# marian42/shapegan

Hardware: AMD Instinct MI355X
Metric: GAN train steps/sec @32^3 voxels (train_wgan.py 5 critic + 1 generator updates, batch 64/GPU) (higher is better)
Workload: dtype f32; 1 GPU; train_wgan.py 32^3 voxel WGAN, fp32, batch=64 synthetic SDF grids (BASELINE configs[1]); global_batch=64, per_gpu_batch=64, parallelism=dp1

## Files before the change

### include/shapegan_hip.h

```cpp
#ifndef SHAPEGAN_HIP_H
#define SHAPEGAN_HIP_H

#include <stddef.h>
#include <stdint.h>

#ifdef __cplusplus
extern "C" {
#endif

#define SG_ABI_VERSION 8

typedef struct ihipStream_t* hipStream_t;

#define SG_ACT_NONE_C 0
#define SG_ACT_LEAKY_C 1
#define SG_ACT_RELU_C 2
#define SG_ACT_TANH_C 3
#define SG_ACT_SIGMOID_C 4

int sg_abi_version(void);
const char* sg_last_error(void);

size_t sg_conv3d_k4s2p1_fwd_workspace_bytes(int batch, int Cin, int Cout, int OD, int OH, int OW);
int sg_conv3d_k4s2p1_fwd(const float* x, const float* w, const float* bias, float* y, int batch, int Cin, int Cin_total,
                         int Cx, int Cout, int ID, int IH, int IW, int act, float slope, void* workspace,
                         size_t workspace_bytes, hipStream_t stream);
int sg_conv3d_k4s2p1_fwd_keep(const float* x, const float* w, const float* bias, float* y, int batch, int Cin, int Cin_total,
                              int Cx, int Cout, int ID, int IH, int IW, int act, float slope, void* workspace,
                              size_t workspace_bytes, int weights_unchanged, hipStream_t stream);
long long sg_conv3d_k4s2p1_image_layout(int kind, const int* dims, size_t workspace_bytes);
int sg_conv3d_k4s2p1_pack_images(int n, const int* kinds, const float* const* weights, void* const* workspaces,
                                 const size_t* workspace_bytes, const int* dims, int* served, hipStream_t stream);
int sg_conv3d_k4s2p1_fwd_impl(const float* x, const float* w, const float* bias, float* y, int batch, int Cin,
                              int Cin_total, int Cx, int Cout, int ID, int IH, int IW, int act, float slope,
                              void* workspace, size_t workspace_bytes, int impl, int debug, hipStream_t stream);
size_t sg_conv3d_k4s2p1_dgrad_workspace_bytes(int Cout, int Cin);
size_t sg_conv3d_k4s2p1_dgrad_workspace_bytes_for(int batch, int Cin, int Cout, int OD, int OH, int OW);
int sg_conv3d_k4s2p1_dgrad(const float* dy, const float* w, const float* bias, float* dx, int batch, int Cin,
                           int Cin_total, int Cx, int Cout, int ID, int IH, int IW, int act, float slope,
                           void* workspace, size_t workspace_bytes, hipStream_t stream);
int sg_conv3d_k4s2p1_dgrad_keep(const float* dy, const float* w, const float* bias, float* dx, int batch, int Cin,
                                int Cin_total, int Cx, int Cout, int ID, int IH, int IW, int act, float slope,
                                void* workspace, size_t workspace_bytes, int weights_unchanged, hipStream_t stream);
int sg_conv3d_k4s2p1_dgrad_impl(const float* dy, const float* w, const float* bias, float* dx, int batch, int Cin,
                                int Cin_total, int Cx, int Cout, int ID, int IH, int IW, int act, float slope,
                                void* workspace, size_t workspace_bytes, int impl, hipStream_t stream);
size_t sg_conv3d_k4s2p1_wgrad_workspace_bytes(int batch, int Cin, int Cout, int OD, int OH, int OW);
int sg_conv3d_k4s2p1_wgrad_impl(const float* dy, const float* x, float* dw, int batch, int Cin, int Cin_total, int Cx,
                                int Cout, int ID, int IH, int IW, void* workspace, size_t workspace_bytes, int impl,
                                hipStream_t stream);
int sg_conv3d_k4s2p1_wgrad(const float* dy, const float* x, float* dw, int batch, int Cin, int Cin_total, int Cx,
                           int Cout, int ID, int IH, int IW, void* workspace, size_t workspace_bytes,
                           hipStream_t stream);
int sg_conv3d_k4s2p1_wgrad_dy_image(int batch, int Cin, int Cout, int OD, int OH, int OW, size_t workspace_bytes, int* mt_total,
                                    long* nslice);
int sg_act_bwd_rowsum_pack8(const float* y, const float* dy, float* dz, float* rowsum, void* dz_image, long N, int C, long nslice,
                            int act, float slope, hipStream_t stream);
int sg_conv3d_k4s2p1_wgrad_prepacked(const float* dy, const float* x, float* dw, int batch, int Cin, int Cin_total, int Cx,
                                     int Cout, int ID, int IH, int IW, void* workspace, size_t workspace_bytes, hipStream_t stream);
int sg_conv3d_k4s2p1_wgrad_act_eligible(int batch, int Cin, int Cout, int OD, int OH, int OW, int act);
int sg_conv3d_k4s2p1_wgrad_act(const float* dy, const float* y, const float* x, float* dw, float* db, int batch, int Cin,
                               int Cin_total, int Cx, int Cout, int ID, int IH, int IW, int act, float slope, void* workspace,
                               size_t workspace_bytes, hipStream_t stream);

int sg_convT3d_k4s2p1_fwd(const float* x, const float* w, const float* bias, float* y, int batch, int Cin_T, int Cout_T,
                          int ID, int IH, int IW, int act, float slope, void* workspace, size_t workspace_bytes,
                          hipStream_t stream);
int sg_convT3d_k4s2p1_to1_pre_eligible(int batch, int C, int ID, int IH, int IW);
int sg_convT3d_k4s2p1_to1_pre(const float* x, const float* w, const float* bias, float* y, const float* in_scale,
                              const float* in_shift, int in_act, float in_slope, int batch, int C, int ID, int IH, int IW, int act,
                              float slope, hipStream_t stream);
int sg_convT3d_k4s2p1_to1_pre_impl(const float* x, const float* w, const float* bias, float* y, const float* in_scale,
                                   const float* in_shift, int in_act, float in_slope, int batch, int C, int ID, int IH, int IW,
                                   int act, float slope, int form, hipStream_t stream);
int sg_convT3d_k4s2p1_to1_pre_grouped(const float* x, const float* w, const float* bias, float* y, const float* in_scale,
                                      const float* in_shift, int in_act, float in_slope, int batch, int C, int ID, int IH, int IW,
                                      int act, float slope, int samples_per_group, long y_group_stride, hipStream_t stream);
int sg_convT3d_k4s2p1_dgrad(const float* dy, const float* w, float* dx, int batch, int Cin_T, int Cout_T, int ID, int IH,
                            int IW, void* workspace, size_t workspace_bytes, hipStream_t stream);
int sg_convT3d_k4s2p1_wgrad(const float* dy, const float* x, float* dw, int batch, int Cin_T, int Cout_T, int ID, int IH,
                            int IW, void* workspace, size_t workspace_bytes, hipStream_t stream);

size_t sg_gemm_workspace_bytes(int M, int N);
int sg_gemm(const float* A, long sai, long sak, const float* B, long sbk, long sbj, float* C, long sci, long scj,
            const float* bias_i, const float* bias_j, int bias_j_shift, int M, int N, int K, int act, float slope,
            void* workspace, size_t workspace_bytes, hipStream_t stream);
#define SG_GEMM_KIND_SKELETON 0
#define SG_GEMM_KIND_GEMM128 1
#define SG_GEMM_KIND_GEMM128_SPLIT 2
#define SG_GEMM_KIND_PERSISTENT 3
#define SG_GEMM_FINALIZE_NONE 0
#define SG_GEMM_FINALIZE_FLAT 1
#define SG_GEMM_FINALIZE_DEEP 2
int sg_gemm_plan(const void* A, long sai, long sak, const void* B, long sbk, long sbj, long sci, long scj, int has_bias_i, int M, int N,
                 int K, const void* workspace, size_t workspace_bytes, long* plan);
int sg_gemm_nt_plan(int batch, int M, int N, long K, long* plan);
size_t sg_gemm_nt_workspace_bytes(int M, int N, long K);
int sg_gemm_nt(const float* A, long lda, const float* B, long ldb, float* C, long ldc, int M, int N, long K, void* workspace,
               size_t workspace_bytes, hipStream_t stream);
// ... 413 lines not shown
```

### shapegan_amd/csrc/conv3d.hip

```cpp
#include "mfma_tile.h"
#include <stdlib.h>

#include "conv_common.h"
#include "../../include/shapegan_hip.h"

namespace sg {

struct PatchCtx {
    int base;
    int mask;
    __device__ __forceinline__ void set(const ConvGeom& g, uint32_t pos) {
        int n, od, oh, ow;
        decode_pos(g, pos, n, od, oh, ow);
        const int id0 = 2 * od - 1, ih0 = 2 * oh - 1, iw0 = 2 * ow - 1;
        base = n * g.Cx * g.ID * g.IH * g.IW + (id0 * g.IH + ih0) * g.IW + iw0;
        int m = 0;
#pragma unroll
        for (int t = 0; t < 4; ++t) {
            if ((unsigned)(id0 + t) < (unsigned)g.ID) m |= 1 << t;
            if ((unsigned)(ih0 + t) < (unsigned)g.IH) m |= 1 << (4 + t);
            if ((unsigned)(iw0 + t) < (unsigned)g.IW) m |= 1 << (8 + t);
        }
        mask = m;
    }
// ... 659 lines not shown

static bool kept_image_of_call(int kind, int batch, int Cin, int Cout, const ConvGeom& g, size_t workspace_bytes, ImageJob* image) {
    if (kind == 0) {
        const HaloFwdPlan p = halo_fwd_plan(batch, Cin, Cout, g, workspace_bytes);
        *image = p.image;
        return p.served;
    }
    const HaloDgradPlan p = halo_dgrad_plan(batch, Cin, Cout, g, workspace_bytes);
    *image = p.image;
    return p.served;
}

int sg_conv3d_k4s2p1_pack_images(int n, const int* kinds, const float* const* weights, void* const* workspaces,
                                 const size_t* workspace_bytes, const int* dims, int* served, hipStream_t stream) {
    SG_CHECK_ARG(n > 0 && n <= 8 && kinds && weights && workspaces && workspace_bytes && dims && served);
    PackJobs jobs;
    for (int i = 0; i < n; ++i) {
        const int* d = dims + 8 * i;
        const int batch = d[0], Cin = d[1], Cin_total = d[2], Cx = d[3], Cout = d[4];
        served[i] = 0;
        SG_CHECK_ARG(weights[i] && batch > 0 && Cin > 0 && Cin <= Cin_total && Cin <= Cx && Cout > 0 && (kinds[i] == 0 || kinds[i] == 1));
        ConvGeom g;
        if (make_geom(g, d[5], d[6], d[7], Cx, Cout)) SG_FAIL(SG_ERR_ARG, "sg_conv3d_k4s2p1_pack_images: bad spatial dims");
        if (check_sizes(g, batch, "sg_conv3d_k4s2p1_pack_images")) return SG_ERR_ARG;
        ImageJob image;
        if (!kept_image_of_call(kinds[i], batch, Cin, Cout, g, workspaces[i] ? workspace_bytes[i] : 0, &image)) continue;
        served[i] = jobs.add(image, weights[i], workspaces[i], Cout, Cin_total, Cin);
    }
    halo_pack_jobs_launch(jobs, stream);
    SG_CHECK_LAUNCH();
    return SG_OK;
}

long long sg_conv3d_k4s2p1_image_layout(int kind, const int* dims, size_t workspace_bytes) {
    if (!dims || (kind != 0 && kind != 1)) return 0;
    const int batch = dims[0], Cin = dims[1], Cin_total = dims[2], Cx = dims[3], Cout = dims[4];
    if (batch <= 0 || Cin <= 1 || Cin > Cin_total || Cin > Cx || Cout <= 0) return 0;
    ConvGeom g;
    if (make_geom(g, dims[5], dims[6], dims[7], Cx, Cout)) return 0;
    if ((long)batch * g.O3() >= (1L << 31) || (long)batch * g.I3() >= (1L << 31)) return 0;
    ImageJob j;
    if (!kept_image_of_call(kind, batch, Cin, Cout, g, workspace_bytes, &j)) return 0;
    unsigned long long h = 1469598103934665603ull;
    const long long f[7] = {j.kind + 1, Cout, Cin_total, Cin, j.nt, (long long)j.offset, 0x5347};
    for (long long v : f)
        for (int b = 0; b < 8; ++b) {
            h ^= (unsigned long long)(v >> (8 * b)) & 0xffull;
            h *= 1099511628211ull;
        }
    h &= 0x7fffffffffffffffull;
    return h ? (long long)h : 1;
}

int sg_conv3d_k4s2p1_dgrad_impl(const float* dy, const float* w, const float* bias, float* dx, int batch, int Cin,
                                int Cin_total, int Cx, int Cout, int ID, int IH, int IW, int act, float slope,
                                void* workspace, size_t workspace_bytes, int impl, hipStream_t stream) {
    HaloDgradForm form;
    SG_CHECK_ARG(dy && w && dx && batch > 0 && Cin > 0 && Cin <= Cin_total && Cin <= Cx && Cout > 0 &&
                 halo_dgrad_form_decode(impl, &form) && form.forced &&
                 (form.ppw == 0 || (!form.one_parity && (form.ppw == 2 || form.ppw == 4 || form.ppw == 8))));
    ConvGeom g;
    if (make_geom(g, ID, IH, IW, Cx, Cout)) SG_FAIL(SG_ERR_ARG, "sg_conv3d_k4s2p1_dgrad_impl: bad spatial dims");
    if (check_sizes(g, batch, "sg_conv3d_k4s2p1_dgrad_impl")) return SG_ERR_ARG;
    const HaloDgradPlan hp = halo_dgrad_plan(batch, Cin, Cout, g, workspace ? workspace_bytes : 0, form);
    if (!hp.served) SG_FAIL(SG_ERR_ARG, "sg_conv3d_k4s2p1_dgrad_impl: shape not eligible for the LDS-halo kernel");
    halo_dgrad_pack(hp, w, Cin, Cin_total, Cout, workspace, stream);
    halo_dgrad_launch(hp, dy, bias, dx, batch, Cin, Cout, g, act, slope, workspace, stream);
    SG_CHECK_LAUNCH();
    return SG_OK;
}

int sg_conv3d_k4s2p1_wgrad_impl(const float* dy, const float* x, float* dw, int batch, int Cin, int Cin_total, int Cx,
                                int Cout, int ID, int IH, int IW, void* workspace, size_t workspace_bytes, int impl,
                                hipStream_t stream) {
    SG_CHECK_ARG(dy && x && dw && batch > 0 && Cin > 0 && Cin <= Cin_total && Cin <= Cx && Cout > 0 && impl == 1);
    ConvGeom g;
    if (make_geom(g, ID, IH, IW, Cx, Cout)) SG_FAIL(SG_ERR_ARG, "sg_conv3d_k4s2p1_wgrad_impl: bad spatial dims");
    if (check_sizes(g, batch, "sg_conv3d_k4s2p1_wgrad_impl")) return SG_ERR_ARG;
    const HaloWgradPlan hp = halo_wgrad_plan(batch, Cin, Cout, g, workspace ? workspace_bytes : 0, true);
    if (!hp.served) SG_FAIL(SG_ERR_ARG, "sg_conv3d_k4s2p1_wgrad_impl: shape not eligible for the LDS-halo kernel");
    halo_wgrad_pack(hp, dy, Cout, g, workspace, stream);
    halo_wgrad_launch(hp, x, dw, Cin, Cin_total, Cout, g, workspace, stream);
    SG_CHECK_LAUNCH();
    return SG_OK;
}

int sg_conv3d_k4s2p1_wgrad_dy_image(int batch, int Cin, int Cout, int OD, int OH, int OW, size_t workspace_bytes, int* mt_total,
                                    long* nslice) {
    if (batch <= 0 || Cin <= 0 || Cout <= 0 || !mt_total || !nslice) return 0;
    ConvGeom g;
    if (make_geom(g, 2 * OD, 2 * OH, 2 * OW, Cin, Cout)) return 0;
    const HaloWgradPlan hp = halo_wgrad_plan(batch, Cin, Cout, g, workspace_bytes, false);
    if (!hp.producer_image) return 0;
    *mt_total = hp.dy_image.nt;
    *nslice = hp.nslice;
    return 1;
}
int sg_act_bwd_rowsum_pack8(const float* y, const float* dy, float* dz, float* rowsum, void* dz_image, long N, int C, long nslice,
                            int act, float slope, hipStream_t stream) {
    SG_CHECK_ARG(y && dy && dz && rowsum && dz_image && N > 0 && C > 0 && C % 128 == 0 && nslice == N * 8);
    SG_CHECK_ARG(act == SG_ACT_LEAKY || act == SG_ACT_RELU);
    SG_CHECK_ARG((((uintptr_t)y | (uintptr_t)dy | (uintptr_t)dz | (uintptr_t)dz_image) & 15) == 0);
    halo_act_bwd_pack8_launch(y, dy, dz, rowsum, dz_image, N * C, C, nslice, act, slope, stream);
    SG_CHECK_LAUNCH();
    return SG_OK;
}
// ... 130 lines not shown
```

### shapegan_amd/csrc/conv3d_halo.hip

```cpp
#include "conv_common.h"

#ifndef SG_RING
#define SG_RING 8
#endif
#ifndef SG_ABLATE
#define SG_ABLATE 0
#endif

namespace sg {

constexpr int kHD = 4, kHH = 18, kHWF = 18;
constexpr int kHWH = 10;
constexpr int kROWH = 2 * kHWH;
constexpr int kROWD = kHH * kROWH;
constexpr int kHS = kHD * kROWD;
constexpr int kCC = 4;

struct HaloFwdArgs {
    const float* x;
    const float4* wp;
    const float* bias;
    float* y;
    ConvGeom g;
    int Cin, Cout;
// ... 1111 lines not shown
#pragma unroll
            for (int i = 0; i < 4; ++i) b[i] = bq[i];
            if (c + 1 < kDCC) {
#pragma unroll
                for (int i = 0; i < 4; ++i) bq[i] = bb[CUR * kDBUF + (c + 1) * kDB + (H0 + i) * BX::PL];
            }
            if (c < kDCC / 2) {
#pragma unroll
                for (int f = 2 * c; f < 2 * c + 2; ++f) fv[f] = buf_load(dres, goff[f], dys + pshift);
            } else {
#pragma unroll
                for (int f = 2 * (c - kDCC / 2); f < 2 * (c - kDCC / 2) + 2; ++f) sdst[NXT * kDBUF + 256 * f] = fv[f];
            }
            __builtin_amdgcn_sched_barrier(0);
            const float av[2][2] = {{a_cur.x, a_cur.y}, {a_cur.z, a_cur.w}};
#pragma unroll
            for (int td = 0; td < 2; ++td)
#pragma unroll
                for (int qd = 0; qd < 4; ++qd) {
                    constexpr int kDead0 = 0, kDead1 = 4;
                    const int hd = qd + 1 - td;
                    if (hd == (PD ? kDead1 : kDead0)) continue;
#pragma unroll
                    for (int rh = 0; rh < 2; ++rh)
                        acc[rh][qd] = __builtin_amdgcn_mfma_f32_16x16x4f32(av[td][rh], b[hd - H0], acc[rh][qd], 0, 0, 0);
                }
            __builtin_amdgcn_sched_barrier(0);
        }
        wcur = wnext;
        __syncthreads();
    };
    auto run_parity = [&](auto pdtag, int par) __attribute__((always_inline)) {
        const bool more = par + 1 < par_end;
        const unsigned wlast = more ? (unsigned)(par + 1) * par_bytes : (unsigned)par * par_bytes + (unsigned)(nstage - 1) * kDCC * 1024u;
        const unsigned dlast = more ? 0u : (unsigned)(nstage - 1) * kDCC * chan_bytes;
        int s = 0;
        for (; s + 1 < nstage; s += 2) {
            stage(IntTag<0>(), pdtag, (unsigned)(s + 1) * kDCC * chan_bytes, wcur + kDCC * 1024u);
            const bool last = s + 2 == nstage;
            if (last && more) set_goff(par + 1);
            stage(IntTag<1>(), pdtag, last ? dlast : (unsigned)(s + 2) * kDCC * chan_bytes, last ? wlast : wcur + kDCC * 1024u);
        }
        if (s < nstage) stage(IntTag<0>(), pdtag, dlast, wlast);
    };
    for (int par = par0; par < par_end; ++par) {
        if ((par >> 2) & 1)
            run_parity(IntTag<1>(), par);
        else
            run_parity(IntTag<0>(), par);
        write_parity(par);
    }
}

size_t halo_dgrad_workspace_bytes(int Cin, int Cout) { return (size_t)8 * ((Cin + 63) / 64) * 64 * Cout * 8 * sizeof(float); }

bool halo_dgrad_form_decode(int impl, HaloDgradForm* form) {
    form->forced = (impl & 1) != 0;
    form->one_parity = (impl & 2) != 0;
    form->ppw = (impl >> 2) & 15;
    form->rows64_dskip = (impl & 64) != 0;
    return (impl & ~127) == 0;
}

HaloDgradPlan halo_dgrad_plan(int batch, int Cin, int Cout, const ConvGeom& g, size_t workspace_bytes, HaloDgradForm form) {
    HaloDgradPlan p = HaloDgradPlan();
    const bool mode1 = g.OD == 4 && g.OH == 4 && g.OW == 4;
    if (!mode1 && (g.OW % 8 != 0 || g.OH % 8 != 0 || g.OD % 2 != 0)) return p;
    if (Cout % 16 != 0 || Cin < 32 || Cin % 8 != 0) return p;
    if (((long)2 * g.Cy * g.OD * g.OH * g.OW + (long)(g.OH + 1) * g.OW + 1) * 4 >= (1L << 26)) return p;
    if (workspace_bytes < halo_dgrad_workspace_bytes(Cin, Cout)) return p;
    if ((long)batch * g.Cy * g.OD * g.OH * g.OW >= (1L << 31)) return p;
    if ((long)2 * g.Cy * g.OD * g.OH * g.OW * 4 >= (long)kBufRange || (long)Cout * 1024 >= (long)kBufRange) return p;
    const int ntw = mode1 ? 1 : g.OW / 8, nth = mode1 ? 1 : g.OH / 8, ntd = mode1 ? 1 : g.OD / 2;
    const long tiles = mode1 ? (batch + 1) / 2 : (long)batch * ntd * nth * ntw;
    const int mtiles = (Cin + 63) / 64;
    if (!form.forced && tiles * mtiles * 8 < (mode1 ? 16 : 64)) return p;
    if (tiles >= (1L << 31) || mtiles > 65535) return p;
    if ((long)8 * mtiles * 2 * Cout * 1024 >= (long)kBufRange) return p;
    int ppw = 8;
    while (ppw > 1 && (tiles * mtiles * (8 / ppw) < 512 || form.one_parity || (Cout / 16) % 2 != 0)) ppw >>= 1;
    if (form.ppw && (Cout / 16) % 2 == 0) ppw = form.ppw;
    const bool r32 = !form.rows64_dskip && (Cin <= 32 || tiles * mtiles * (8 / ppw) < 256);
    const bool dskip = mode1 && !r32 && (!form.forced || form.rows64_dskip);
    if (form.rows64_dskip && !dskip) return p;
    p.served = true;
    p.kernel = dskip ? HaloDgradKernel::dskip4
                     : (mode1 ? (r32 ? HaloDgradKernel::rows32_4 : HaloDgradKernel::rows64_4)
                              : (r32 ? HaloDgradKernel::rows32 : HaloDgradKernel::rows64));
    p.grid = dim3((unsigned)tiles, r32 ? (unsigned)((Cin + 31) / 32) : (unsigned)mtiles, 8 / ppw);
    p.block = 256;
    p.lds = (size_t)2 * 16 * 256 * sizeof(float);
    {
        const long wgs = tiles * mtiles * (8 / ppw);
        const long cost2 = ((wgs + 511) / 512) * 2, cost3 = ((wgs + 767) / 768) * 3;
        if (cost2 <= cost3) p.lds = 56 * 1024;
    }
    p.image = ImageJob{dskip ? 3 : 1, mtiles * 2, 0};
    p.workspace_need = halo_dgrad_workspace_bytes(Cin, Cout);
    p.mtiles = mtiles;
    p.ppw = ppw;
    p.ntd = ntd;
    p.nth = nth;
    p.ntw = ntw;
    return p;
}

void halo_dgrad_pack(const HaloDgradPlan& p, const float* w, int Cin, int Cin_total, int Cout, void* workspace, hipStream_t stream) {
    const long total = 8L * p.image.nt * Cout * 64;
    int blocks = (int)((total + 255) / 256);
    if (blocks > 4096) blocks = 4096;
    hipLaunchKernelGGL(pack_dgrad_frag_kernel, dim3(blocks), dim3(256), 0, stream, w, workspace_at<float4>(workspace, p.image.offset), Cout,
                       Cin_total, Cin, p.image.nt, p.image.kind >> 1);
}

static HaloDgradArgs halo_dgrad_args(const HaloDgradPlan& p, const float* dy, const float* bias, float* dx, int batch, int Cin, int Cout,
                                     const ConvGeom& g, int act, float slope, void* workspace) {
    HaloDgradArgs a;
    a.dy = dy;
    a.wp = workspace_at<float4>(workspace, p.image.offset);
    a.bias = bias;
    a.dx = dx;
    a.g = g;
    a.Cin = Cin;
    a.Cout = Cout;
    a.mtiles = p.mtiles;
    a.batch = batch;
    a.ppw = p.ppw;
    a.dntw = FastDiv(p.ntw);
    a.dnth = FastDiv(p.nth);
    a.dntd = FastDiv(p.ntd);
    a.act = act;
    a.slope = slope;
    return a;
}

void halo_dgrad_launch(const HaloDgradPlan& p, const float* dy, const float* bias, float* dx, int batch, int Cin, int Cout,
                       const ConvGeom& g, int act, float slope, void* workspace, hipStream_t stream) {
    const HaloDgradArgs a = halo_dgrad_args(p, dy, bias, dx, batch, Cin, Cout, g, act, slope, workspace);
    switch (p.kernel) {
    case HaloDgradKernel::dskip4:
        hipLaunchKernelGGL(conv_dgrad_halo_dskip_kernel, p.grid, dim3(p.block), p.lds, stream, a);
        break;
    case HaloDgradKernel::rows32_4:
        hipLaunchKernelGGL((conv_dgrad_halo32_kernel<1>), p.grid, dim3(p.block), p.lds, stream, a);
        break;
    case HaloDgradKernel::rows64_4:
        hipLaunchKernelGGL((conv_dgrad_halo_kernel<1>), p.grid, dim3(p.block), p.lds, stream, a);
        break;
    case HaloDgradKernel::rows32:
        hipLaunchKernelGGL((conv_dgrad_halo32_kernel<0>), p.grid, dim3(p.block), p.lds, stream, a);
        break;
    case HaloDgradKernel::rows64:
        hipLaunchKernelGGL((conv_dgrad_halo_kernel<0>), p.grid, dim3(p.block), p.lds, stream, a);
        break;
    }
}


constexpr int kWROWD = 368;
constexpr int kWHS = kHD * kWROWD;
constexpr int kWNF = (2 * kHD * kHH + 7) / 8;
constexpr int kWROWD_SKIP = 364;

struct HaloWgradArgs {
    const float4* ap;
    const float* x;
    float* ws;
    ConvGeom g;
    int Cin, Cout, nslice, per_split, mt_total;
    long ldw;
    FastDiv dntw, dnth, dOD;
};

__global__ void __launch_bounds__(256) pack_wgrad_dy_kernel(const float* __restrict__ dy, float4* __restrict__ ap,
                                                            ConvGeom g, int Cout, int MT, int nslice, FastDiv dntw,
                                                            FastDiv dnth, FastDiv dOD) {
    const long total = (long)MT * nslice * 8 * 64;
    const long O3 = (long)g.OD * g.OH * g.OW;
    for (long e = (long)blockIdx.x * 256 + threadIdx.x; e < total; e += (long)gridDim.x * 256) {
        const int lane = (int)(e & 63);
        const int gq = (int)((e >> 6) & 7);
        const long q = e >> 9;
        const uint32_t sl = (uint32_t)(q % nslice);
        const int mt = (int)(q / nslice);
        uint32_t twi, thi, od, n, q1, q2;
        dntw.divmod(sl, q1, twi);
        dnth.divmod(q1, q2, thi);
        dOD.divmod(q2, n, od);
        const int co = mt * 32 + (lane & 31);
        float4 v = make_float4(0.f, 0.f, 0.f, 0.f);
        if (co < Cout) {
            const float* src = dy + ((long)n * Cout + co) * O3 + ((long)od * g.OH + (thi * 8 + gq)) * g.OW + twi * 8 + (lane >> 5);
            v = make_float4(src[0], src[2], src[4], src[6]);
        }
        ap[e] = v;
    }
}

template <int NCH, int V>
__device__ __forceinline__ void conv_wgrad_halo_body(const HaloWgradArgs& a) {
    constexpr bool SKIP = V >= 0;
    static_assert(!SKIP || NCH == 2, "the static-skip column map is the 2-channel form's");
    constexpr int WROWD = SKIP ? kWROWD_SKIP : kWROWD;
    constexpr int WHS = kHD * WROWD;
    extern __shared__ __attribute__((aligned(16))) float wbox[];
    const int tid = threadIdx.x, lane = tid & 63;
// ... 575 lines not shown
```

### shapegan_amd/csrc/conv_common.h

```cpp
#pragma once
#include "common.h"

namespace sg {

struct FastDiv {
    uint32_t m, s, d;
    FastDiv() : m(0), s(0), d(1) {}
    explicit FastDiv(uint32_t dd) : d(dd) {
        s = 0;
        while ((1u << s) < dd) ++s;
        m = (uint32_t)((((uint64_t)1 << 32) * (((uint64_t)1 << s) - dd)) / dd + 1);
    }
    __device__ __forceinline__ uint32_t div(uint32_t n) const { return (__umulhi(n, m) + n) >> s; }
    __device__ __forceinline__ void divmod(uint32_t n, uint32_t& q, uint32_t& r) const {
        q = div(n);
        r = n - q * d;
    }
};

struct ConvGeom {
    int ID, IH, IW;
    int OD, OH, OW;
    int Cx, Cy;
    FastDiv dOW, dOH, dOD;
// ... 25 lines not shown
    g.dOW = FastDiv(g.OW);
    g.dOH = FastDiv(g.OH);
    g.dOD = FastDiv(g.OD);
    return 0;
}



struct KernelPlan {
    bool served;
    dim3 grid;
    unsigned block;
    size_t lds;
    size_t workspace_need;
};
template <class T>
static inline T* workspace_at(void* workspace, size_t offset) { return reinterpret_cast<T*>(static_cast<char*>(workspace) + offset); }

struct ImageJob {
    int kind;
    int nt;
    size_t offset;
};

struct PackJob {
    const float* w;
    float4* wp;
    int kind, Cout, Cin_total, Cin, nt;
};
struct PackJobs {
    PackJob job[8];
    int n = 0;
    int add(const ImageJob& image, const float* w, void* workspace, int Cout, int Cin_total, int Cin) {
        if (n >= 8) return 0;
        job[n++] = PackJob{w, workspace_at<float4>(workspace, image.offset), image.kind, Cout, Cin_total, Cin, image.nt};
        return 1;
    }
};
int halo_pack_jobs_launch(const PackJobs& jobs, hipStream_t stream);

struct HaloFwdForm {
    bool forced;
    int variant;
    bool keep_lds;
    bool keep_rows128;
    bool dskip;
};
HaloFwdForm halo_fwd_form_decode(int debug);
struct HaloDgradForm {
    bool forced;
    bool one_parity;
    int ppw;
    bool rows64_dskip;
};
bool halo_dgrad_form_decode(int impl, HaloDgradForm* form);

size_t halo_fwd_workspace_bytes(int Cin, int Cout);
constexpr int kHaloFwd4MaxSplit = 8;
enum class HaloFwdKernel { halo4, halo4_dskip, rows128_w8, rows128_w4, rows64 };
struct HaloFwdPlan : KernelPlan {
    HaloFwdKernel kernel;
    ImageJob image;
    int nth, ntw;
    int csplit;
    size_t partial_offset;
};
HaloFwdPlan halo_fwd_plan(int batch, int Cin, int Cout, const ConvGeom& g, size_t workspace_bytes, HaloFwdForm form = HaloFwdForm());
void halo_fwd_pack(const HaloFwdPlan& p, const float* w, int Cin, int Cin_total, int Cout, void* workspace, hipStream_t stream);
void halo_fwd_launch(const HaloFwdPlan& p, const float* x, const float* bias, float* y, int batch, int Cin, int Cout, const ConvGeom& g,
                     int act, float slope, void* workspace, hipStream_t stream);

size_t halo_dgrad_workspace_bytes(int Cin, int Cout);
enum class HaloDgradKernel { dskip4, rows32_4, rows64_4, rows32, rows64 };
struct HaloDgradPlan : KernelPlan {
    HaloDgradKernel kernel;
    ImageJob image;
    int mtiles, ppw;
    int ntd, nth, ntw;
};
HaloDgradPlan halo_dgrad_plan(int batch, int Cin, int Cout, const ConvGeom& g, size_t workspace_bytes, HaloDgradForm form = HaloDgradForm());
void halo_dgrad_pack(const HaloDgradPlan& p, const float* w, int Cin, int Cin_total, int Cout, void* workspace, hipStream_t stream);
void halo_dgrad_launch(const HaloDgradPlan& p, const float* dy, const float* bias, float* dx, int batch, int Cin, int Cout,
                       const ConvGeom& g, int act, float slope, void* workspace, hipStream_t stream);

enum class HaloWgradKernel { halo4, rows64, rows128_skip_h, rows128 };
struct HaloWgradPlan : KernelPlan {
    HaloWgradKernel kernel;
    ImageJob dy_image;
    bool producer_image;
    int nslice, nsplit, per_split, mtiles;
    size_t partial_offset;
};
HaloWgradPlan halo_wgrad_plan(int batch, int Cin, int Cout, const ConvGeom& g, size_t workspace_bytes, bool forced);
void halo_wgrad_pack(const HaloWgradPlan& p, const float* dy, int Cout, const ConvGeom& g, void* workspace, hipStream_t stream);
void halo_wgrad_launch(const HaloWgradPlan& p, const float* x, float* dw, int Cin, int Cin_total, int Cout, const ConvGeom& g,
                       void* workspace, hipStream_t stream);
int halo_act_bwd_pack8_launch(const float* y, const float* dy, float* dz, float* rowsum, void* ap, long rows, int C, long nslice,
                              int act, float slope, hipStream_t stream);

enum class EdgeFwdKernel { lds_staged, gather };
struct EdgeFwdPlan : KernelPlan {
    EdgeFwdKernel kernel;
    int nt, actk;
    int bh, units_per_wg;
};
EdgeFwdPlan edge_fwd_plan(int batch, int Cin, int Cout, const ConvGeom& g, int act, float slope);
void edge_fwd_launch(const EdgeFwdPlan& p, const float* x, const float* w, const float* bias, float* y, int batch, int Cin_total,
                     int Cout, const ConvGeom& g, int act, float slope, hipStream_t stream);

struct EdgeWgradPlan : KernelPlan {
    int nt, fuse;
};
EdgeWgradPlan edge_wgrad_plan(int batch, int Cin, int Cout, const ConvGeom& g, size_t workspace_bytes, int fuse_act);
void edge_wgrad_launch(const EdgeWgradPlan& p, const float* dy, const float* y, const float* x, float* dw, float* db, int batch,
                       int Cin_total, int Cout, const ConvGeom& g, float slope, void* workspace, hipStream_t stream);

enum class EdgeDgradKernel { walk_one_pair, walk_all_taps, plane_fused, tap_planes };
struct EdgeDgradPlan : KernelPlan {
    EdgeDgradKernel kernel;
    int splits;
};
EdgeDgradPlan edge_dgrad_walk_plan(int form, int batch, int Cin, int Cout, const ConvGeom& g);
EdgeDgradPlan edge_dgrad_plan(int batch, int Cin, int Cout, const ConvGeom& g, size_t workspace_bytes);
void edge_dgrad_launch(const EdgeDgradPlan& p, const float* dy, const float* w, const float* bias, float* dx, int batch, int Cin_total,
                       int Cout, const ConvGeom& g, int act, float slope, void* workspace, hipStream_t stream,
                       const float* in_scale = nullptr, const float* in_shift = nullptr, int in_act = 0, float in_slope = 0.f,
// ... 4 lines not shown
```

### shapegan_amd/csrc_cpu/shapegan_cpu.cpp

```cpp
#include <math.h>
#include <stdint.h>
#include <stdio.h>
#include <string.h>

#include <algorithm>
#include <vector>

#include "../../include/shapegan_hip.h"

typedef void* hipStream_t_;
#define SG_OK 0
#define SG_ERR_ARG (-1)
#define SG_ERR_WORKSPACE (-3)
enum { ACT_NONE = 0, ACT_LEAKY = 1, ACT_RELU = 2, ACT_TANH = 3, ACT_SIGMOID = 4 };

static thread_local char g_err[512];
#define CPU_CHECK(cond)                                                                  \
    do {                                                                                 \
        if (!(cond)) {                                                                   \
            snprintf(g_err, sizeof(g_err), "%s: bad argument: %s", __func__, #cond);     \
            return SG_ERR_ARG;                                                           \
        }                                                                                \
    } while (0)

// ... 91 lines not shown
                            }
                        }
            }
            if (act != ACT_NONE)
                for (long e = 0; e < I3; ++e) xo[e] = apply_act(xo[e], act, slope);
        }
    return SG_OK;
}

int sg_conv3d_k4s2p1_wgrad_cpu(const float* dy, const float* x, float* dw, int batch, int Cin, int Cin_total, int Cx, int Cout,
                               int ID, int IH, int IW, void*, size_t, void*) {
    CPU_CHECK(dy && x && dw && batch > 0 && Cin > 0 && Cin <= Cin_total && Cin <= Cx && Cout > 0 && !(ID & 1) && !(IH & 1) && !(IW & 1));
    const int OD = ID / 2, OH = IH / 2, OW = IW / 2;
    const long I3 = (long)ID * IH * IW, O3 = (long)OD * OH * OW;
#pragma omp parallel for collapse(2) schedule(static)
    for (int co = 0; co < Cout; ++co)
        for (int ci = 0; ci < Cin; ++ci) {
            double acc[64];
            for (int k = 0; k < 64; ++k) acc[k] = 0.0;
            for (int n = 0; n < batch; ++n) {
                const float* yo = dy + ((long)n * Cout + co) * O3;
                const float* xi = x + ((long)n * Cx + ci) * I3;
                for (int kd = 0; kd < 4; ++kd)
                    for (int kh = 0; kh < 4; ++kh)
                        for (int kw = 0; kw < 4; ++kw) {
                            const int ow0 = kw == 0 ? 1 : 0, ow1 = kw == 3 ? OW - 1 : OW;
                            float s = 0.f;
                            for (int od = 0; od < OD; ++od) {
                                const int id = 2 * od + kd - 1;
                                if ((unsigned)id >= (unsigned)ID) continue;
                                for (int oh = 0; oh < OH; ++oh) {
                                    const int ih = 2 * oh + kh - 1;
                                    if ((unsigned)ih >= (unsigned)IH) continue;
                                    const float* xr = xi + ((long)id * IH + ih) * IW + kw - 1;
                                    const float* yr = yo + ((long)od * OH + oh) * OW;
                                    float r = 0.f;
                                    for (int ow = ow0; ow < ow1; ++ow) r += yr[ow] * xr[2 * ow];
                                    s += r;
                                }
                            }
                            acc[kd * 16 + kh * 4 + kw] += (double)s;
                        }
            }
            float* d = dw + ((long)co * Cin_total + ci) * 64;
            for (int k = 0; k < 64; ++k) d[k] = (float)acc[k];
        }
    return SG_OK;
}

int sg_conv3d_k4s2p1_dgrad_keep_cpu(const float* dy, const float* w, const float* bias, float* dx, int batch, int Cin,
                                    int Cin_total, int Cx, int Cout, int ID, int IH, int IW, int act, float slope, void* ws,
                                    size_t wb, int, void* st) {
    return sg_conv3d_k4s2p1_dgrad_cpu(dy, w, bias, dx, batch, Cin, Cin_total, Cx, Cout, ID, IH, IW, act, slope, ws, wb, st);
}
int sg_conv3d_k4s2p1_fwd_keep_cpu(const float* x, const float* w, const float* bias, float* y, int batch, int Cin, int Cin_total,
                                  int Cx, int Cout, int ID, int IH, int IW, int act, float slope, void* ws, size_t wb, int, void* st) {
    return sg_conv3d_k4s2p1_fwd_cpu(x, w, bias, y, batch, Cin, Cin_total, Cx, Cout, ID, IH, IW, act, slope, ws, wb, st);
}
int sg_conv3d_k4s2p1_pack_images_cpu(int n, const int* kinds, const float* const* weights, void* const* workspaces,
                                     const size_t* workspace_bytes, const int* dims, int* served, void*) {
    CPU_CHECK(n > 0 && n <= 8 && kinds && weights && workspaces && workspace_bytes && dims && served);
    for (int i = 0; i < n; ++i) served[i] = 0;
    return SG_OK;
}
int sg_act_bwd_rowsum_pack8_cpu(const float* y, const float* dy, float* dz, float* rowsum, void*, long N, int C, long, int act,
                                float slope, void*) {
    CPU_CHECK(y && dy && dz && rowsum && N > 0 && C > 0);
    for (long r = 0; r < N * C; ++r) {
        double s = 0;
        for (int e = 0; e < 512; ++e) {
            const float v = act_grad_out(y[r * 512 + e], dy[r * 512 + e], act, slope);
            dz[r * 512 + e] = v;
            s += (double)v;
        }
        rowsum[r] = (float)s;
    }
    return SG_OK;
}
int sg_conv3d_k4s2p1_wgrad_prepacked_cpu(const float* dy, const float* x, float* dw, int batch, int Cin, int Cin_total, int Cx,
                                         int Cout, int ID, int IH, int IW, void* ws, size_t wb, void* st) {
    return sg_conv3d_k4s2p1_wgrad_cpu(dy, x, dw, batch, Cin, Cin_total, Cx, Cout, ID, IH, IW, ws, wb, st);
}
int sg_convT3d_k4s2p1_fwd_cpu(const float* x, const float* w, const float* bias, float* y, int batch, int Cin_T, int Cout_T,
                              int ID, int IH, int IW, int act, float slope, void* ws, size_t wb, void* st) {
    return sg_conv3d_k4s2p1_dgrad_cpu(x, w, bias, y, batch, Cout_T, Cout_T, Cout_T, Cin_T, 2 * ID, 2 * IH, 2 * IW, act, slope, ws,
                                      wb, st);
}
int sg_convT3d_k4s2p1_to1_pre_cpu(const float* x, const float* w, const float* bias, float* y, const float* in_scale,
                                  const float* in_shift, int in_act, float in_slope, int batch, int C, int ID, int IH, int IW,
                                  int act, float slope, void* st) {
    CPU_CHECK(x && w && y && in_scale && in_shift && batch > 0 && C > 0 && C <= 64 && IH * IW <= 256);
    CPU_CHECK(in_act == ACT_NONE || in_act == ACT_LEAKY || in_act == ACT_RELU);
    const long S = (long)ID * IH * IW, total = (long)batch * C * S;
    std::vector<float> t((size_t)total);
#pragma omp parallel for schedule(static)
    for (long e = 0; e < total; ++e) {
        const int c = (int)((e / S) % C);
        t[(size_t)e] = apply_act(x[e] * in_scale[c] + in_shift[c], in_act, in_slope);
    }
    return sg_conv3d_k4s2p1_dgrad_cpu(t.data(), w, bias, y, batch, 1, 1, 1, C, 2 * ID, 2 * IH, 2 * IW, act, slope, nullptr, 0, st);
}
int sg_convT3d_k4s2p1_to1_pre_grouped_cpu(const float* x, const float* w, const float* bias, float* y, const float* in_scale,
                                          const float* in_shift, int in_act, float in_slope, int batch, int C, int ID, int IH,
                                          int IW, int act, float slope, int spg, long y_group_stride, void* st) {
    CPU_CHECK(spg > 0 && batch % spg == 0);
    const long S = (long)ID * IH * IW;
// ... 3210 lines not shown
```

### shapegan_amd/ops.py

```python
import contextlib
import ctypes
import weakref

import numpy as np
import torch
from torch.autograd import Function
from torch.autograd.function import once_differentiable

from . import lib as L
from .lib import ACT_LEAKY, ACT_NONE, ACT_RELU, ACT_SIGMOID, ACT_TANH, check, f32c, ptr, stream, workspace


def _lib():
    return L.load()


def conv_fwd_raw(x, w, bias, act=ACT_NONE, slope=0.0, keep=False):
    N, Cx, D, H, W = x.shape
    Co, Ct = w.shape[0], w.shape[1]
    if Cx > Ct:
        raise RuntimeError("conv: input has %d channels, weight expects %d" % (Cx, Ct))
    ptr(x)
    L.reset_call_state()
    y = torch.empty((N, Co, D // 2, H // 2, W // 2), dtype=torch.float32, device=x.device)
# ... 94 lines not shown
        return bool(served[0])

    def register_group(self, weights):
        refs = [weakref.ref(w) for w in weights]
        for w in weights:
            self.groups[id(w)] = (refs, weakref.ref(w))


_KEPT = _KeptWeightImages()


def invalidate_weight_images():
    L.bump_param_epoch()


def register_pack_group(weights):
    _KEPT.register_group(list(weights))


def conv_dgrad_raw(dy, w, bias, cin, act=ACT_NONE, slope=0.0, keep=False, out=None):
    N, Co, OD, OH, OW = dy.shape
    Ct = w.shape[1]
    if w.shape[0] != Co or cin > Ct:
        raise RuntimeError("conv dgrad: shape mismatch")
    shape = (N, cin, 2 * OD, 2 * OH, 2 * OW)
    if out is not None:
        if tuple(out.shape) != shape or out.dtype != torch.float32 or not out.is_contiguous() or out.device != dy.device:
            raise RuntimeError("conv dgrad: `out` must be a contiguous fp32 tensor of shape %s on %s" % (shape, dy.device))
        dx = out
    else:
        dx = torch.empty(shape, dtype=torch.float32, device=dy.device)
    lib = _lib()
    nb = lib.sg_conv3d_k4s2p1_dgrad_workspace_bytes_for(N, cin, Co, OD, OH, OW)
    if keep and cin > 1 and dy.is_cuda and L.writers_known(w) and not torch.cuda.is_current_stream_capturing():
        ws, unchanged = _KEPT.get(w, nb, (N, cin, Ct, cin, Co, 2 * OD, 2 * OH, 2 * OW), kind=1)
        check(lib.sg_conv3d_k4s2p1_dgrad_keep(ptr(dy), ptr(w), ptr(bias), ptr(dx), N, cin, Ct, cin, Co, 2 * OD, 2 * OH, 2 * OW,
                                              act, slope, ptr(ws), ws.numel(), int(unchanged), stream()), "conv3d_dgrad_keep")
        return dx
    ws = workspace("dgrad", nb, dy.device)
    check(lib.sg_conv3d_k4s2p1_dgrad(ptr(dy), ptr(w), ptr(bias), ptr(dx), N, cin, Ct, cin, Co, 2 * OD, 2 * OH, 2 * OW,
                                     act, slope, ptr(ws), ws.numel(), stream()), "conv3d_dgrad")
    return dx


def conv_dgrad_halo_raw(dy, w, bias, cin, act=ACT_NONE, slope=0.0, impl=1):
    N, Co, OD, OH, OW = dy.shape
    Ct = w.shape[1]
    dx = torch.empty((N, cin, 2 * OD, 2 * OH, 2 * OW), dtype=torch.float32, device=dy.device)
    lib = _lib()
    ws = workspace("dgrad", lib.sg_conv3d_k4s2p1_dgrad_workspace_bytes(Co, cin), dy.device)
    check(lib.sg_conv3d_k4s2p1_dgrad_impl(ptr(dy), ptr(w), ptr(bias), ptr(dx), N, cin, Ct, cin, Co, 2 * OD, 2 * OH,
                                          2 * OW, act, slope, ptr(ws), ws.numel(), impl, stream()), "conv3d_dgrad_impl")
    return dx


_WGRAD_WS_CAP = 256 << 20


def _param_grad_out(param, shape, device):
    dst = L.grad_destination(param, shape) if param is not None else None
    return dst if dst is not None else torch.empty(shape, dtype=torch.float32, device=device)


def conv_wgrad_raw(dy, x, ct, out=None):
    N, Co, OD, OH, OW = dy.shape
    Cx = x.shape[1]
    if x.shape[0] != N or x.shape[2] != 2 * OD:
        raise RuntimeError("conv wgrad: shape mismatch")
    if out is not None:
        dw = out
        if Cx < ct:
            dw.zero_()
    elif Cx < ct:
        dw = torch.zeros((Co, ct, 4, 4, 4), dtype=torch.float32, device=dy.device)
    else:
        dw = torch.empty((Co, ct, 4, 4, 4), dtype=torch.float32, device=dy.device)
    lib = _lib()
    nb = min(lib.sg_conv3d_k4s2p1_wgrad_workspace_bytes(N, Cx, Co, OD, OH, OW), _WGRAD_WS_CAP)
    ws = workspace("splitk", nb, dy.device)
    check(lib.sg_conv3d_k4s2p1_wgrad(ptr(dy), ptr(x), ptr(dw), N, Cx, ct, Cx, Co, 2 * OD, 2 * OH, 2 * OW, ptr(ws),
                                     ws.numel(), stream()), "conv3d_wgrad")
    return dw


def _wgrad_dy_image(N, Cx, Co, O, device):
    if device.type != "cuda":
        return None
    lib = _lib()
    nb = min(lib.sg_conv3d_k4s2p1_wgrad_workspace_bytes(N, Cx, Co, O, O, O), _WGRAD_WS_CAP)
    ws = workspace("splitk", nb, device)
    mt, ns = ctypes.c_int(0), ctypes.c_long(0)
    if not lib.sg_conv3d_k4s2p1_wgrad_dy_image(N, Cx, Co, O, O, O, ws.numel(), ctypes.byref(mt), ctypes.byref(ns)):
        return None
    return ws, mt.value, ns.value


def conv_wgrad_prepacked_raw(dy, x, ct, ws, out=None):
    N, Co = dy.shape[0], dy.shape[1]
    Cx = x.shape[1]
    dw = out if out is not None else torch.empty((Co, ct, 4, 4, 4), dtype=torch.float32, device=dy.device)
    if Cx < ct:
        raise RuntimeError("conv_wgrad_prepacked: partial input channels are not served")
    check(_lib().sg_conv3d_k4s2p1_wgrad_prepacked(ptr(dy), ptr(x), ptr(dw), N, Cx, ct, Cx, Co, x.shape[2], x.shape[3], x.shape[4],
                                                  ptr(ws), ws.numel(), stream()), "conv3d_wgrad_prepacked")
    return dw

# ... 2316 lines not shown
```

Before: 62.82 steps/s.

## Add depth-walking halo dgrad kernel for OD=8 transposed-conv backward

Adds a new halo dgrad kernel that walks all eight output parities along depth within one workgroup, covering half the depth per block. It reuses a preloaded bitmask of dy gather offsets and a register ring of weight loads, and writes paired outputs with 64-bit stores. The planner picks it by default for OD=8 shapes with enough workgroups. The aim is fewer workgroups, better dy/weight reuse and fewer store instructions, at the cost of register pressure and a less parallel grid. A query API reporting the chosen dgrad form is also added.

```diff
diff --git a/include/shapegan_hip.h b/include/shapegan_hip.h
--- a/include/shapegan_hip.h
+++ b/include/shapegan_hip.h
@@ -45,6 +45,14 @@
 int sg_conv3d_k4s2p1_dgrad_impl(const float* dy, const float* w, const float* bias, float* dx, int batch, int Cin,
                                 int Cin_total, int Cx, int Cout, int ID, int IH, int IW, int act, float slope,
                                 void* workspace, size_t workspace_bytes, int impl, hipStream_t stream);
+#define SG_DGRAD_FORM_NONE 0
+#define SG_DGRAD_FORM_DSKIP4 1
+#define SG_DGRAD_FORM_ROWS32_4 2
+#define SG_DGRAD_FORM_ROWS64_4 3
+#define SG_DGRAD_FORM_ROWS32 4
+#define SG_DGRAD_FORM_ROWS64 5
+#define SG_DGRAD_FORM_DEPTH_WALK 6
+int sg_conv3d_k4s2p1_dgrad_form(int batch, int Cin, int Cout, int OD, int OH, int OW, size_t workspace_bytes);
 size_t sg_conv3d_k4s2p1_wgrad_workspace_bytes(int batch, int Cin, int Cout, int OD, int OH, int OW);
 int sg_conv3d_k4s2p1_wgrad_impl(const float* dy, const float* x, float* dw, int batch, int Cin, int Cin_total, int Cx,
                                 int Cout, int ID, int IH, int IW, void* workspace, size_t workspace_bytes, int impl,
diff --git a/shapegan_amd/csrc/conv3d.hip b/shapegan_amd/csrc/conv3d.hip
--- a/shapegan_amd/csrc/conv3d.hip
+++ b/shapegan_amd/csrc/conv3d.hip
@@ -735,6 +735,19 @@
     return h ? (long long)h : 1;
 }
 
+int sg_conv3d_k4s2p1_dgrad_form(int batch, int Cin, int Cout, int OD, int OH, int OW, size_t workspace_bytes) {
+    static_assert((int)HaloDgradKernel::dskip4 + 1 == SG_DGRAD_FORM_DSKIP4 && (int)HaloDgradKernel::rows32_4 + 1 == SG_DGRAD_FORM_ROWS32_4 &&
+                  (int)HaloDgradKernel::rows64_4 + 1 == SG_DGRAD_FORM_ROWS64_4 && (int)HaloDgradKernel::rows32 + 1 == SG_DGRAD_FORM_ROWS32 &&
+                  (int)HaloDgradKernel::rows64 + 1 == SG_DGRAD_FORM_ROWS64 && (int)HaloDgradKernel::rows64_dwalk + 1 == SG_DGRAD_FORM_DEPTH_WALK,
+                  "SG_DGRAD_FORM_* mirror HaloDgradKernel");
+    ConvGeom g;
+    if (batch <= 0 || Cin <= 1 || Cout <= 0 || !query_geom(g, Cin, Cout, OD, OH, OW)) return SG_DGRAD_FORM_NONE;
+    if ((long)batch * g.O3() >= (1L << 31) || (long)batch * g.I3() >= (1L << 31)) return SG_DGRAD_FORM_NONE;
+    if (edge_dgrad_plan(batch, Cin, Cout, g, workspace_bytes).served) return SG_DGRAD_FORM_NONE;
+    const HaloDgradPlan hp = halo_dgrad_plan(batch, Cin, Cout, g, workspace_bytes);
+    return hp.served ? 1 + (int)hp.kernel : SG_DGRAD_FORM_NONE;
+}
+
 int sg_conv3d_k4s2p1_dgrad_impl(const float* dy, const float* w, const float* bias, float* dx, int batch, int Cin,
                                 int Cin_total, int Cx, int Cout, int ID, int IH, int IW, int act, float slope,
                                 void* workspace, size_t workspace_bytes, int impl, hipStream_t stream) {
diff --git a/shapegan_amd/csrc/conv3d_halo.hip b/shapegan_amd/csrc/conv3d_halo.hip
--- a/shapegan_amd/csrc/conv3d_halo.hip
+++ b/shapegan_amd/csrc/conv3d_halo.hip
@@ -1187,6 +1187,213 @@
     }
 }
 
+__global__ void __launch_bounds__(256) __attribute__((amdgpu_waves_per_eu(2))) conv_dgrad_halo_dwalk_kernel(HaloDgradArgs a) {
+    constexpr int NTN = 2;
+    constexpr int kDCC = 16, kDNF = 16, kDBUF = kDNF * 256;
+    using BX = DBox<0>;
+    constexpr int kDB = BX::CH;
+    extern __shared__ __attribute__((aligned(16))) float box[];
+    const int hf = blockIdx.x & 1, ph = blockIdx.z;
+    uint32_t twi, thi, n, q1;
+    a.dntw.divmod(blockIdx.x >> 1, q1, twi);
+    a.dnth.divmod(q1, n, thi);
+    const int qd0 = hf * 4, qh0 = thi * 8, qw0 = twi * 8;
+    const int qd0e = hf ? a.g.OD - 2 : 0;
+    const int ci0 = blockIdx.y * 64;
+
+    const int tid = threadIdx.x, lane = tid & 63;
+    const int wave = __builtin_amdgcn_readfirstlane(tid >> 6);
+    const int wm = wave >> 1, wn = wave & 1, r = lane & 31, kpar = lane >> 5;
+    const int lanebase = wn * BX::TNOFF + (r >> 3) * BX::BW + (r & 7) + 1 - kpar;
+
+    f32x16 acc[NTN];
+#pragma unroll
+    for (int t = 0; t < NTN; ++t)
+#pragma unroll
+        for (int q = 0; q < 16; ++q) acc[t][q] = 0.f;
+
+    lds_float* const bl = (lds_float*)box;
+    const lds_float* bb = bl + lanebase;
+    pin_vgpr(bb);
+    lds_float* sdst = bl + tid;
+    pin_vgpr(sdst);
+
+    const int G = a.Cout;
+    const unsigned par_bytes = (unsigned)(a.mtiles * 2) * (unsigned)G * 1024u;
+    const __amdgpu_buffer_rsrc_t wres = make_rsrc(a.wp + ((long)(blockIdx.y * 2 + wm) * G) * 64);
+    const unsigned wvoff = lane * 16;
+
+    const int O3 = a.g.OD * a.g.OH * a.g.OW;
+    const int obias = (a.g.OH + 1) * a.g.OW + 1;
+    const __amdgpu_buffer_rsrc_t dres = __builtin_amdgcn_make_buffer_rsrc(
+        const_cast<float*>(a.dy + (long)n * a.g.Cy * O3 - obias), 0, 1 << 26, 0x00020000);
+    const unsigned chan_bytes = (unsigned)O3 * 4u;
+    const unsigned pair_bytes = (unsigned)(2 * a.g.OH * a.g.OW) * 4u;
+    unsigned gword[kDNF], goff[kDNF];
+#pragma unroll
+    for (int f = 0; f < kDNF; ++f) {
+        const int e = tid + 256 * f;
+        const int ci = e / kDB;
+        const int rem = e - ci * kDB;
+        const int hd = rem / BX::PL, hh = (rem - hd * BX::PL) / BX::BW, hw = rem % BX::BW;
+        const int od = qd0 - 1 + hd, ode = qd0e - 1 + hd, oh = qh0 - 1 + hh, ow = qw0 - 1 + hw;
+        const bool never = e >= kDCC * kDB;
+        const unsigned cls = (ode < 0 ? 1u << 26 : 0u) | (ode + 1 >= a.g.OD ? 1u << 27 : 0u) | (oh < 0 ? 1u << 28 : 0u) |
+                             (oh + 1 >= a.g.OH ? 1u << 29 : 0u) | (ow < 0 ? 1u << 30 : 0u) | (ow + 1 >= a.g.OW ? 1u << 31 : 0u);
+        const int off0 = ci * O3 + (od * a.g.OH + oh) * a.g.OW + ow + obias;
+        gword[f] = never ? 0xffffffffu : ((unsigned)off0 * 4u) | cls;
+        pin_vgpr(gword[f]);
+    }
+    unsigned pshift = 0;
+    auto set_goff = [&](int i) __attribute__((always_inline)) {
+        const int pair = i >> 2, pd = (i >> 1) & 1, pw = i & 1;
+        const bool dedge = pair == hf;
+        const unsigned mask = 0x03ffffffu | (dedge ? (pd ? 1u << 27 : 1u << 26) : 0u) | (ph ? 1u << 29 : 1u << 28) | (pw ? 1u << 31 : 1u << 30);
+#pragma unroll
+        for (int f = 0; f < kDNF; ++f) goff[f] = gword[f] & mask;
+        pshift = (unsigned)((pd * a.g.OH + ph) * a.g.OW + pw) * 4u + (unsigned)pair * pair_bytes;
+    };
+    const long I3 = (long)a.g.ID * a.g.IH * a.g.IW;
+    const __amdgpu_buffer_rsrc_t ores = make_rsrc(a.dx + (long)n * a.g.Cx * I3);
+    const __amdgpu_buffer_rsrc_t bres = make_rsrc(a.bias ? a.bias : a.dx);
+    unsigned ovoff[NTN];
+#pragma unroll
+    for (int tn = 0; tn < NTN; ++tn) {
+        const int qd = qd0 + tn, qh = qh0 + wn * 4 + (r >> 3), qw = qw0 + (r & 7);
+        ovoff[tn] = (unsigned)(((2 * qd) * a.g.IH + 2 * qh) * a.g.IW + 2 * qw + 4 * kpar * (int)I3) * 4u;
+        pin_vgpr(ovoff[tn]);
+    }
+    const unsigned bvoff = kpar * 16;
+    const unsigned opair_bytes = (unsigned)(4 * a.g.IH * a.g.IW) * 4u;
+    float keep[NTN][16];
+#pragma unroll
+    for (int t = 0; t < NTN; ++t)
+#pragma unroll
+        for (int q = 0; q < 16; ++q) keep[t][q] = 0.f;
+    auto write_pass = [&](int i) __attribute__((always_inline)) {
+        const int pair = i >> 2, pd = (i >> 1) & 1, pw = i & 1;
+        const unsigned oshift = (unsigned)((pd * a.g.IH + ph) * a.g.IW) * 4u + (unsigned)pair * opair_bytes;
+        if (pw == 0) {
+#pragma unroll
+            for (int q = 0; q < 16; ++q) {
+                const int cis = ci0 + wm * 32 + (q & 3) + 8 * (q >> 2);
+                const float bv = a.bias && cis < a.Cin ? buf_load(bres, bvoff, (unsigned)cis * 4u) : 0.f;
+#pragma unroll
+                for (int tn = 0; tn < NTN; ++tn) keep[tn][q] = sg_apply_act(acc[tn][q] + bv, a.act, a.slope);
+            }
+        } else {
+            typedef unsigned u32x2 __attribute__((ext_vector_type(2)));
+#pragma unroll
+            for (int q = 0; q < 16; ++q) {
+                const int cis = ci0 + wm * 32 + (q & 3) + 8 * (q >> 2);
+                if (cis < a.Cin) {
+                    const float bv = a.bias ? buf_load(bres, bvoff, (unsigned)cis * 4u) : 0.f;
+#pragma unroll
+                    for (int tn = 0; tn < NTN; ++tn) {
+                        u32x2 v;
+                        v.x = __builtin_bit_cast(unsigned, keep[tn][q]);
+                        v.y = __builtin_bit_cast(unsigned, sg_apply_act(acc[tn][q] + bv, a.act, a.slope));
+                        __builtin_amdgcn_raw_buffer_store_b64(v, ores, (int)ovoff[tn], (int)((unsigned)cis * (unsigned)I3 * 4u + oshift), 0);
+                    }
+                }
+            }
+        }
+#pragma unroll
+        for (int t = 0; t < NTN; ++t)
+#pragma unroll
+            for (int q = 0; q < 16; ++q) acc[t][q] = 0.f;
+    };
+    auto pass_weights = [&](int i) __attribute__((always_inline)) {
+        return (unsigned)(4 * ((i >> 1) & 1) + 2 * ph + (i & 1)) * par_bytes;
+    };
+
+    set_goff(0);
+    float fv[kDNF];
+    constexpr int kRing = 8;
+    float4 aring[kRing];
+    unsigned wcur = pass_weights(0);
+#pragma unroll
+    for (int f = 0; f < kDNF; ++f) fv[f] = buf_load(dres, goff[f], pshift);
+#pragma unroll
+    for (int u = 0; u < kRing; ++u) aring[u] = buf_load4(wres, wvoff, wcur + (unsigned)u * 1024u);
+#pragma unroll
+    for (int f = 0; f < kDNF; ++f) sdst[256 * f] = fv[f];
+    __syncthreads();
+
+    constexpr int O00 = BX::PL + BX::BW, O01 = BX::PL, O10 = BX::BW, O11 = 0;
+    const int nstage = a.Cout / kDCC;
+    auto stage = [&](auto tag, auto edgetag, unsigned dys, unsigned wnext) __attribute__((always_inline)) {
+        constexpr int CUR = decltype(tag)::value, NXT = CUR ^ 1, EDGE = decltype(edgetag)::value;
+        constexpr int kOff[4] = {O00, O01, O10, O11};
+        float bq[NTN][4];
+#pragma unroll
+        for (int tn = 0; tn < NTN; ++tn)
+#pragma unroll
+            for (int j = 0; j < 4; ++j)
+                if (!((EDGE == 1 && tn == 0 && j >= 2) || (EDGE == 2 && tn == 1 && j < 2))) bq[tn][j] = bb[CUR * kDBUF + tn * BX::PL + kOff[j]];
+        __builtin_amdgcn_sched_barrier(0);
+#pragma unroll
+        for (int c = 0; c < kDCC; ++c) {
+            const float4 a_cur = aring[c % kRing];
+            aring[c % kRing] = c + kRing < kDCC ? buf_load4(wres, wvoff, wcur + (unsigned)(c + kRing) * 1024u)
+                                                : buf_load4(wres, wvoff, wnext + (unsigned)(c + kRing - kDCC) * 1024u);
+            float b[NTN][4];
+#pragma unroll
+            for (int tn = 0; tn < NTN; ++tn)
+#pragma unroll
+                for (int j = 0; j < 4; ++j)
+                    if (!((EDGE == 1 && tn == 0 && j >= 2) || (EDGE == 2 && tn == 1 && j < 2))) b[tn][j] = bq[tn][j];
+            if (c + 1 < kDCC) {
+#pragma unroll
+                for (int tn = 0; tn < NTN; ++tn)
+#pragma unroll
+                    for (int j = 0; j < 4; ++j)
+                        if (!((EDGE == 1 && tn == 0 && j >= 2) || (EDGE == 2 && tn == 1 && j < 2)))
+                            bq[tn][j] = bb[CUR * kDBUF + (c + 1) * kDB + tn * BX::PL + kOff[j]];
+            }
+            if (c < kDCC / 2) {
+#pragma unroll
+                for (int f = 2 * c; f < 2 * c + 2; ++f) fv[f] = buf_load(dres, goff[f], dys + pshift);
+            } else {
+#pragma unroll
+                for (int f = 2 * (c - kDCC / 2); f < 2 * (c - kDCC / 2) + 2; ++f) sdst[NXT * kDBUF + 256 * f] = fv[f];
+            }
+            __builtin_amdgcn_sched_barrier(0);
+            const float av[4] = {a_cur.x, a_cur.y, a_cur.z, a_cur.w};
+#pragma unroll
+            for (int j = 0; j < 4; ++j)
+#pragma unroll
+                for (int tn = 0; tn < NTN; ++tn)
+                    if (!((EDGE == 1 && tn == 0 && j >= 2) || (EDGE == 2 && tn == 1 && j < 2)))
+                        acc[tn] = __builtin_amdgcn_mfma_f32_32x32x2f32(av[j], b[tn][j], acc[tn], 0, 0, 0);
+            __builtin_amdgcn_sched_barrier(0);
+        }
+        wcur = wnext;
+        __syncthreads();
+    };
+    auto run_pass = [&](auto edgetag, int i) __attribute__((always_inline)) {
+        const bool more = i + 1 < 8;
+        const unsigned wlast = more ? pass_weights(i + 1) : pass_weights(i) + (unsigned)(nstage - 1) * kDCC * 1024u;
+        const unsigned dlast = more ? 0u : (unsigned)(nstage - 1) * kDCC * chan_bytes;
+        for (int s = 0; s + 1 < nstage; s += 2) {
+            stage(IntTag<0>(), edgetag, (unsigned)(s + 1) * kDCC * chan_bytes, wcur + kDCC * 1024u);
+            const bool last = s + 2 == nstage;
+            if (last && more) set_goff(i + 1);
+            stage(IntTag<1>(), edgetag, last ? dlast : (unsigned)(s + 2) * kDCC * chan_bytes, last ? wlast : wcur + kDCC * 1024u);
+        }
+    };
+    for (int i = 0; i < 8; ++i) {
+        const bool edge = hf ? i >= 6 : i < 2;
+        if (!edge)
+            run_pass(IntTag<0>(), i);
+        else if (hf == 0)
+            run_pass(IntTag<1>(), i);
+        else
+            run_pass(IntTag<2>(), i);
+        write_pass(i);
+    }
+}
+
 size_t halo_dgrad_workspace_bytes(int Cin, int Cout) { return (size_t)8 * ((Cin + 63) / 64) * 64 * Cout * 8 * sizeof(float); }
 
 bool halo_dgrad_form_decode(int impl, HaloDgradForm* form) {
@@ -1194,7 +1401,8 @@
     form->one_parity = (impl & 2) != 0;
     form->ppw = (impl >> 2) & 15;
     form->rows64_dskip = (impl & 64) != 0;
-    return (impl & ~127) == 0;
+    form->depth_walk = (impl & 128) != 0;
+    return (impl & ~255) == 0;
 }
 
 HaloDgradPlan halo_dgrad_plan(int batch, int Cin, int Cout, const ConvGeom& g, size_t workspace_bytes, HaloDgradForm form) {
@@ -1218,22 +1426,27 @@
     const bool r32 = !form.rows64_dskip && (Cin <= 32 || tiles * mtiles * (8 / ppw) < 256);
     const bool dskip = mode1 && !r32 && (!form.forced || form.rows64_dskip);
     if (form.rows64_dskip && !dskip) return p;
+    const long walk_tiles = (long)batch * nth * ntw * 2;
+    const bool walk_shape = !mode1 && g.OD == 8 && Cin > 32 && (Cout / 16) % 2 == 0 && walk_tiles < (1L << 31);
+    if (form.depth_walk && (!walk_shape || form.ppw || form.one_parity || form.rows64_dskip)) return p;
+    const bool dwalk = walk_shape && (form.forced ? form.depth_walk : walk_tiles * mtiles * 2 >= 512);
     p.served = true;
     p.kernel = dskip ? HaloDgradKernel::dskip4
                      : (mode1 ? (r32 ? HaloDgradKernel::rows32_4 : HaloDgradKernel::rows64_4)
-                              : (r32 ? HaloDgradKernel::rows32 : HaloDgradKernel::rows64));
-    p.grid = dim3((unsigned)tiles, r32 ? (unsigned)((Cin + 31) / 32) : (unsigned)mtiles, 8 / ppw);
+                              : (dwalk ? HaloDgradKernel::rows64_dwalk : (r32 ? HaloDgradKernel::rows32 : HaloDgradKernel::rows64)));
+    p.grid = dwalk ? dim3((unsigned)walk_tiles, (unsigned)mtiles, 2)
+                   : dim3((unsigned)tiles, r32 ? (unsigned)((Cin + 31) / 32) : (unsigned)mtiles, 8 / ppw);
     p.block = 256;
     p.lds = (size_t)2 * 16 * 256 * sizeof(float);
     {
-        const long wgs = tiles * mtiles * (8 / ppw);
+        const long wgs = dwalk ? walk_tiles * mtiles * 2 : tiles * mtiles * (8 / ppw);
         const long cost2 = ((wgs + 511) / 512) * 2, cost3 = ((wgs + 767) / 768) * 3;
         if (cost2 <= cost3) p.lds = 56 * 1024;
     }
     p.image = ImageJob{dskip ? 3 : 1, mtiles * 2, 0};
     p.workspace_need = halo_dgrad_workspace_bytes(Cin, Cout);
     p.mtiles = mtiles;
-    p.ppw = ppw;
+    p.ppw = dwalk ? 8 : ppw;
     p.ntd = ntd;
     p.nth = nth;
     p.ntw = ntw;
@@ -1287,6 +1500,9 @@
         break;
     case HaloDgradKernel::rows64:
         hipLaunchKernelGGL((conv_dgrad_halo_kernel<0>), p.grid, dim3(p.block), p.lds, stream, a);
+        break;
+    case HaloDgradKernel::rows64_dwalk:
+        hipLaunchKernelGGL(conv_dgrad_halo_dwalk_kernel, p.grid, dim3(p.block), p.lds, stream, a);
         break;
     }
 }
diff --git a/shapegan_amd/csrc/conv_common.h b/shapegan_amd/csrc/conv_common.h
--- a/shapegan_amd/csrc/conv_common.h
+++ b/shapegan_amd/csrc/conv_common.h
@@ -101,6 +101,7 @@
     bool one_parity;
     int ppw;
     bool rows64_dskip;
+    bool depth_walk;
 };
 bool halo_dgrad_form_decode(int impl, HaloDgradForm* form);
 
@@ -120,7 +121,7 @@
                      int act, float slope, void* workspace, hipStream_t stream);
 
 size_t halo_dgrad_workspace_bytes(int Cin, int Cout);
-enum class HaloDgradKernel { dskip4, rows32_4, rows64_4, rows32, rows64 };
+enum class HaloDgradKernel { dskip4, rows32_4, rows64_4, rows32, rows64, rows64_dwalk };
 struct HaloDgradPlan : KernelPlan {
     HaloDgradKernel kernel;
     ImageJob image;
diff --git a/shapegan_amd/csrc_cpu/shapegan_cpu.cpp b/shapegan_amd/csrc_cpu/shapegan_cpu.cpp
--- a/shapegan_amd/csrc_cpu/shapegan_cpu.cpp
+++ b/shapegan_amd/csrc_cpu/shapegan_cpu.cpp
@@ -167,6 +167,9 @@
                                     int Cin_total, int Cx, int Cout, int ID, int IH, int IW, int act, float slope, void* ws,
                                     size_t wb, int, void* st) {
     return sg_conv3d_k4s2p1_dgrad_cpu(dy, w, bias, dx, batch, Cin, Cin_total, Cx, Cout, ID, IH, IW, act, slope, ws, wb, st);
+}
+int sg_conv3d_k4s2p1_dgrad_form_cpu(int, int, int, int, int, int, size_t) {
+    return 0;
 }
 int sg_conv3d_k4s2p1_fwd_keep_cpu(const float* x, const float* w, const float* bias, float* y, int batch, int Cin, int Cin_total,
                                   int Cx, int Cout, int ID, int IH, int IW, int act, float slope, void* ws, size_t wb, int, void* st) {
diff --git a/shapegan_amd/ops.py b/shapegan_amd/ops.py
--- a/shapegan_amd/ops.py
+++ b/shapegan_amd/ops.py
@@ -170,6 +170,12 @@
     check(lib.sg_conv3d_k4s2p1_dgrad_impl(ptr(dy), ptr(w), ptr(bias), ptr(dx), N, cin, Ct, cin, Co, 2 * OD, 2 * OH,
                                           2 * OW, act, slope, ptr(ws), ws.numel(), impl, stream()), "conv3d_dgrad_impl")
     return dx
+
+
+def conv_dgrad_form(batch, cin, cout, ogrid):
+    lib = L._load_hip()
+    nb = lib.sg_conv3d_k4s2p1_dgrad_workspace_bytes_for(batch, cin, cout, *ogrid)
+    return lib.sg_conv3d_k4s2p1_dgrad_form(batch, cin, cout, *ogrid, nb)
 
 
 _WGRAD_WS_CAP = 256 << 20
```

New measurement: 63.50 steps/s (median of 6 runs). +1.1%, better.
